# mattayes/tigerbeetle

Measured on AMD Instinct MI355X. Metric: transfers/sec committed (whole node, bit-exact results) + p99 batch latency, higher is better.
Workload: dtype u128

## Files before the change

### tigerbeetle_amd/csrc/engine.hip

```cpp
#include <hip/hip_runtime.h>

#include <algorithm>
#include <atomic>
#include <chrono>
#include <cmath>
#include <cstdarg>
#include <cstdio>
#include <cstdlib>
#include <cstring>
#include <numeric>
#include <string>
#include <vector>
#include <map>
#include <functional>
#include <mutex>

#include "../../include/tbgpu.h"
#include "../../include/tbgpu_bench.h"
#include "../../include/tbgpu_shard.h"
#include "k_apply.h"
#include "k_flow.h"
#include "k_aux.h"
#include "k_replay.h"
#include "k_route.h"
// ... 899 lines not shown
    if (E->wb.read_done) (void)hipEventDestroy(E->wb.read_done);
    if (E->wb.captured) (void)hipEventDestroy(E->wb.captured);
    for (hipEvent_t e : E->event_pool) (void)hipEventDestroy(e);
    if (E->pf_done) (void)hipEventDestroy(E->pf_done);
    for (int i = 0; i < 16; i++) if (E->markers[i]) (void)hipEventDestroy(E->markers[i]);
    if (E->stream) (void)hipStreamDestroy(E->stream);
    delete E;
}

extern "C" int tbgpu_reset(tbgpu_t* E) {
    API_ENTER(E, false);
    if (E->node) return node_api_reset(E->node);
    E->pf_input = E->pf_claim = nullptr;
    E->poisoned = false;
    HIPCK(hipSetDevice(E->device));
    if (E->wb.inflight) {
        HIPCK(hipStreamSynchronize(E->stream));
        HIPCK(hipStreamSynchronize(E->wb.stream));
        E->wb.inflight = E->wb.copying = E->wb.counts_known = E->wb.tail = false;
    }
    E->ckpt_valid = false;
    E->ckpt_scan = false;
    std::vector<u64>().swap(E->ckpt_ids);
    return engine_clear(E);
}

static int engine_sync(tbgpu* E) {
    HIPCK(hipMemcpyAsync(E->h_globals, E->g, sizeof(Globals), hipMemcpyDeviceToHost, E->stream));
    HIPCK(hipStreamSynchronize(E->stream));
    const Globals g = *E->h_globals;
    E->commit_ts = g.commit_timestamp;
    E->pending = false;
    int st = prof_collect(E);
    if (st) return st;
    if (g.panic) {
        E->poisoned = true;
        return fail(TBGPU_STATUS_PANIC, "device panic 0x%llx (the reference would have trapped)", (unsigned long long)g.panic);
    }
    return TBGPU_STATUS_OK;
}

static int enqueue_call(tbgpu* E, u8 op, u32 nb, const u64* h_off, const u8* events_dev, u32* results_dev,
                        u32* reply_bytes_dev, bool routed = false, u8* codes = nullptr, u32 cert_ext = 0,
                        const u8* events_src = nullptr, const u64* d_meta = nullptr,
                        const OwnerLegArgs* owner = nullptr, const u64* inline_meta = nullptr,
                        const NodeImport* imp = nullptr, const u64* ev_ts = nullptr) {
    const u64* d_off = d_meta ? d_meta : E->meta;
    const u64* d_ts = d_off + (nb + 1);
    u32 b0 = 0;
    while (b0 < nb) {
        u32 b1 = b0;
        while (b1 < nb && b1 - b0 < E->pb_max && h_off[b1 + 1] - h_off[b0] <= E->pe_max) b1++;
        if (b1 == b0) return fail(TBGPU_STATUS_INVALID, "batch larger than pass_events_max");
        const u64 n = h_off[b1] - h_off[b0];
        E->epoch++;
        if (E->epoch == 0) {
            HIPCK(hipMemsetAsync(E->T.account_mark, 0, E->account_cap * sizeof(u32), E->stream));
            E->epoch = 1;
            E->dedup_force = true;
        }
        PassArgs P{};
        P.op = op;
        P.epoch = E->epoch;
        P.b0 = b0;
        P.b1 = b1;
        P.e0 = h_off[b0];
        P.n = (u32)n;
        P.batch_off = d_off;
        P.batch_ts = d_ts;
        P.events = events_dev;
        P.events_src = events_src;
        P.results = results_dev;
        P.reply_bytes = reply_bytes_dev;
        P.info = E->info;
        P.eflags = E->eflags;
        P.dr = E->dr;
        P.cr = E->cr;
        P.ps = E->ps;
        P.rs = E->rs;
        P.amt = E->amt;
        P.amt_hi = E->amt + E->pe_max;
        P.kid = E->kid;
        P.kpid = E->kpid;
        P.dep_list = E->dep_list;
        P.dep_count = E->dep_count;
        P.dedup = E->dedup;
        P.dedup_mask = std::min<u64>(pow2_at_least(std::max<u64>(4 * n, 64)), E->dedup_cap) - 1;
        P.sum_shards = E->sum_shards;
        P.pass_words = E->sum_shards;
        P.log_base = E->log_next;
        P.T = E->T;
        P.ablate = E->ablate;
        P.routed = routed ? 1 : 0;
        P.codes = codes;
        P.cert_ext = cert_ext;
        P.seq_pv = E->balances_set ? 1u : 0u;
        P.ev_ts = ev_ts;
        P.inplace = E->inplace_call ? 1u : 0u;
        P.legs = (op == OP_CREATE_TRANSFERS && E->legs_ok && b1 - b0 <= LEG_PREPARES_MAX && n >= E->legs_min &&
                  !(E->ablate & ABL_LEGS) && !owner) ? 1 : 0;
        P.apply_late = (op == OP_CREATE_TRANSFERS && !P.legs) ? 1 : 0;
        P.leg_shift = E->leg_shift;
        P.leg_buckets = E->leg_buckets;
        P.resolve_slow = P.legs && E->lean_ok ? E->resolve_slow : nullptr;
        P.leg_w = E->leg_w;
        P.leg_off = E->leg_off;
        P.leg_tot = E->leg_tot;
        const bool flow = op == OP_CREATE_TRANSFERS && E->flow_ok && !E->balances_set && !(E->ablate & ABL_FLOW) &&
                          b1 - b0 <= FLOW_NB_MAX && !owner;
        P.flow_words = E->flow_ok ? E->F.words : nullptr;
        P.late_in_flow = (flow && (P.apply_late || P.legs)) ? 1u : 0u;

        P.kclock = nullptr;
        if (E->profile && !E->kclock_off && (E->prof_mask & ((1u << K_VALIDATE) | (1u << K_RESOLVE) | (1u << K_APPLY) | (1u << K_SPANS))) &&
            E->kclock_next < KCLOCK_SLOTS) {
            const u32 slot = E->kclock_next++;
            P.kclock = E->kclock + (u64)slot * KCLOCK_WORDS;
            E->kclock_used.push_back({slot, (n > 0 ? 1u : 0u) | 2u | (P.legs ? 4u : 0u)});
        }

        ProfilePair pass_pp;
        int st = prof_begin(E, &pass_pp, K_PASS);
        if (st) return st;
        ProfilePair pp;
        if ((st = prof_begin(E, &pp, K_CLEAR))) return st;
        const u64 clear_n = E->dedup_force ? E->dedup_cap : E->dedup_prev;
        const u32 clear_grid = (u32)std::min<u64>(1024, std::max<u64>(1, clear_n / 2048));
        u64* meta_dst = inline_meta && b0 == 0 ? (u64*)d_off : nullptr;
        ImportGate gate{};
        if (imp && n > 0) gate = ImportGate{imp->count, imp->room, 0, imp->flag};
        hipLaunchKernelGGL(tb_pass_clear, dim3(clear_grid), dim3(256), 0, E->stream, E->dedup, E->dedup_cap, E->sum_shards,
                           E->g, E->epoch, E->dedup_force ? 1u : 0u, E->leg_tot, E->leg_buckets, meta_dst,
                           inline_meta ? inline_meta[0] : 0, inline_meta ? inline_meta[1] : 0, inline_meta ? inline_meta[2] : 0,
                           P.kclock, gate, imp && b0 == 0 ? imp->leg_counts : nullptr,
                           imp && b0 == 0 ? imp->legs_n : 0u);
        HIPCK(hipGetLastError());
        E->dedup_force = false;
        E->dedup_prev = P.dedup_mask + 1;
        if ((st = prof_end(E, &pp))) return st;

        if (imp && n > 0) {
            const u32 ig = (u32)std::min<u64>(4096, (n + 255) / 256);
            hipLaunchKernelGGL(tb_node_import_flush, dim3((u32)std::min<u64>(1024, (E->account_cap + 255) / 256)), dim3(256), 0,
                               E->stream, E->T, E->account_cap, imp->N.world, imp->self, (const u32*)imp->flag);
            hipLaunchKernelGGL(tb_node_import, dim3(ig), dim3(256), 0, E->stream, E->T, imp->N, events_dev + P.e0 * 128, n,
                               imp->self, imp->count, imp->os_of);
            HIPCK(hipGetLastError());
        }
        if (n > 0) {
            if ((st = prof_begin(E, &pp, K_VALIDATE))) return st;
            const u32 grid = (u32)((n + VALIDATE_THREADS - 1) / VALIDATE_THREADS);
            if (op == OP_CREATE_TRANSFERS) {
                if (P.events_src) {
                    hipLaunchKernelGGL(tb_transfers_validate<true>, dim3(grid), dim3(VALIDATE_THREADS), 0, E->stream, P);
                } else {
                    hipLaunchKernelGGL(tb_transfers_validate<false>, dim3(grid), dim3(VALIDATE_THREADS), 0, E->stream, P);
                }
            } else {
                if (P.events_src) {
                    hipLaunchKernelGGL(tb_accounts_validate<true>, dim3(grid), dim3(VALIDATE_THREADS), 0, E->stream, P);
                } else {
                    hipLaunchKernelGGL(tb_accounts_validate<false>, dim3(grid), dim3(VALIDATE_THREADS), 0, E->stream, P);
                }
            }
            HIPCK(hipGetLastError());
            if (E->wb.copying) HIPCK(hipEventRecord(E->wb.read_done, E->stream));
            if ((st = prof_end(E, &pp))) return st;
        }
        if ((st = prof_begin(E, &pp, K_RESOLVE))) return st;
        if (op == OP_CREATE_TRANSFERS) {
            if (P.resolve_slow) {
                hipLaunchKernelGGL(tb_resolve_lean, dim3(b1 - b0), dim3(RESOLVE_THREADS), 0, E->stream, P);
            }
            hipLaunchKernelGGL(tb_resolve<OP_CREATE_TRANSFERS>, dim3(b1 - b0), dim3(RESOLVE_THREADS), 0, E->stream, P);
        } else {
            hipLaunchKernelGGL(tb_resolve<OP_CREATE_ACCOUNTS>, dim3(b1 - b0), dim3(RESOLVE_THREADS), 0, E->stream, P);
        }
        HIPCK(hipGetLastError());
        if ((st = prof_end(E, &pp))) return st;
        if (P.legs || P.apply_late) {
            if ((st = prof_begin(E, &pp, K_APPLY))) return st;
            if (P.legs) {
                hipLaunchKernelGGL(tb_apply_legs, dim3(E->leg_buckets + APPLY_EXTRA), dim3(APPLY_THREADS),
                                   tb_apply_lds_bytes(E->leg_shift, b1 - b0), E->stream, P);
            }
            if (n > 0 && !owner && !P.late_in_flow) {
                const u32 grid = (u32)std::min<u64>((n + 255) / 256, P.legs ? 2048 : 1u << 20);
                hipLaunchKernelGGL(tb_apply_events, dim3(grid), dim3(256), 0, E->stream, P);
            }
            HIPCK(hipGetLastError());
            if ((st = prof_end(E, &pp))) return st;
        }
        if ((st = prof_begin(E, &pp, K_REPLAY))) return st;
        if (flow) {
            UndoEntry* seq_undo = E->undo;
            u32 seq_cap = E->undo_cap;
            FlowArgs F = E->F;
            F.grid = flow_grid(E);

            if (n <= 65536) F.grid = std::min<u32>(F.grid, std::max<u32>(4, (u32)((n + 511) / 512)));
            if (E->flow_launch) F.grid = E->flow_launch;
            hipLaunchKernelGGL(tb_flow, dim3(F.grid), dim3(FLOW_THREADS), 0, E->stream, P, F, seq_undo, seq_cap);
        } else if (op == OP_CREATE_TRANSFERS) {
            hipLaunchKernelGGL(tb_replay<OP_CREATE_TRANSFERS>, dim3(1), dim3(REPLAY_THREADS), 0, E->stream, P,
                               E->undo, E->undo_cap);
        } else {
            hipLaunchKernelGGL(tb_replay<OP_CREATE_ACCOUNTS>, dim3(1), dim3(REPLAY_THREADS), 0, E->stream, P,
                               E->undo, E->undo_cap);
        }
        HIPCK(hipGetLastError());
        if ((st = prof_end(E, &pp))) return st;
        if (owner && n > 0) {
            hipLaunchKernelGGL(tb_owner_legs, dim3((u32)((n + 255) / 256)), dim3(256), 0, E->stream, P, *owner);
            HIPCK(hipGetLastError());
        }
        if (imp && imp->ev_legs) HIPCK(hipEventRecord((hipEvent_t)imp->ev_legs, E->stream));
        if ((st = prof_end(E, &pass_pp))) return st;
        E->passes++;
        E->events += n;
        if (op == OP_CREATE_TRANSFERS) E->log_next += n;
        b0 = b1;
    }
    return TBGPU_STATUS_OK;
}

static int prepare_call(tbgpu* E, u8 op, u32 nb, const u64* timestamps, const u32* lens, u64 floor_ts,
                        u64* total_events, bool upload = true) {
    if (op != OP_CREATE_ACCOUNTS && op != OP_CREATE_TRANSFERS) {
        return fail(TBGPU_STATUS_INVALID, "operation %u is not a create operation", op);
    }
    if (nb == 0) return fail(TBGPU_STATUS_INVALID, "no batches");
    if (nb > E->meta_cap) return fail(TBGPU_STATUS_INVALID, "too many batches in one call (%u > %llu)", nb,
                                      (unsigned long long)E->meta_cap);
    if (E->pending) {
        int st = engine_sync(E);
        if (st) return st;
    }
    u64* h_off = E->h_meta;
    u64* h_ts = E->h_meta + (nb + 1);
    u64 prev = floor_ts;
    h_off[0] = 0;
    for (u32 k = 0; k < nb; k++) {
        const u64 ts = timestamps[k];
        const u32 L = lens[k];
        if (L > BATCH_EVENTS_MAX) return fail(TBGPU_STATUS_INVALID, "batch %u has %u events (max %u)", k, L, BATCH_EVENTS_MAX);
        if (!(ts > prev)) return fail(TBGPU_STATUS_PANIC, "timestamp %llu <= commit timestamp %llu",
                                      (unsigned long long)ts, (unsigned long long)prev);
        if (L > 0) {
            if (ts < L) return fail(TBGPU_STATUS_PANIC, "timestamp %llu < batch length %u", (unsigned long long)ts, L);
            if (!(ts - L + 1 > prev)) return fail(TBGPU_STATUS_PANIC, "first event timestamp <= commit timestamp");
        }
        prev = ts;
        h_off[k + 1] = h_off[k] + L;
        h_ts[k] = ts;
    }
    if (op == OP_CREATE_TRANSFERS && E->log_next + h_off[nb] > E->xlog_cap) {
        return fail(TBGPU_STATUS_INVALID, "transfer log full (%llu + %llu events > capacity %llu)",
                    (unsigned long long)E->log_next, (unsigned long long)h_off[nb], (unsigned long long)E->xlog_cap);
    }
    if (upload) HIPCK(hipMemcpyAsync(E->meta, E->h_meta, (2 * (u64)nb + 1) * 8, hipMemcpyHostToDevice, E->stream));
    E->last_batch_ts = prev;
    *total_events = h_off[nb];
    return TBGPU_STATUS_OK;
}

static int commit_lookup(tbgpu* E, bool accounts, const void* input, uint32_t input_len, void* output,
                         uint32_t output_cap, uint32_t* out_len) {
    if (input_len % 16 != 0) return fail(TBGPU_STATUS_INVALID, "lookup body not a multiple of 16");
    const u32 n = input_len / 16;
    if (n > E->lookup_cap) return fail(TBGPU_STATUS_INVALID, "too many ids");
    if (n == 0) return TBGPU_STATUS_OK;
    HIPCK(hipMemcpyAsync(E->lookup_ids, input, input_len, hipMemcpyHostToDevice, E->stream));
    if (accounts) {
        hipLaunchKernelGGL(tb_lookup<true>, dim3((n + 255) / 256), dim3(256), 0, E->stream, E->T, E->lookup_ids, n,
                           E->lookup_out, E->lookup_found);
    } else {
        hipLaunchKernelGGL(tb_lookup<false>, dim3((n + 255) / 256), dim3(256), 0, E->stream, E->T, E->lookup_ids, n,
                           E->lookup_out, E->lookup_found);
    }
    HIPCK(hipGetLastError());
    std::vector<u8> found(n);
    std::vector<u8> recs((u64)n * 128);
    HIPCK(hipMemcpyAsync(found.data(), E->lookup_found, n, hipMemcpyDeviceToHost, E->stream));
    HIPCK(hipMemcpyAsync(recs.data(), E->lookup_out, (u64)n * 128, hipMemcpyDeviceToHost, E->stream));
    HIPCK(hipStreamSynchronize(E->stream));
    const u32 slots = output_cap / 128;
    u32 m = 0;
    for (u32 i = 0; i < n; i++) {
        if (found[i] && m < slots) {
            memcpy((u8*)output + (u64)m * 128, recs.data() + (u64)i * 128, 128);
            m++;
        }
    }
    *out_len = m * 128;
    return TBGPU_STATUS_OK;
}

static int wb_pump(tbgpu* E, u64 budget, hipEvent_t after);

static int commit_host(tbgpu* E, u8 op, u32 n, const uint64_t* timestamps, const void* const* inputs,
                       const uint32_t* input_lens, void* const* outputs, uint32_t* out_lens, const uint32_t* out_caps) {
    const void* claim = E->pf_claim;
    E->pf_claim = nullptr;
    std::vector<u32> lens(n);
    for (u32 k = 0; k < n; k++) {
        if (input_lens[k] % 128 != 0) return fail(TBGPU_STATUS_INVALID, "create body not a multiple of 128");
        lens[k] = input_lens[k] / 128;
        if (out_caps && (u64)out_caps[k] < (u64)lens[k] * 8) return fail(TBGPU_STATUS_INVALID, "output too small");
    }
// ... 2487 lines not shown
```

### tigerbeetle_amd/csrc/k_validate.h

```cpp
#pragma once

#include "pass.h"

#define TB_CODE_PANIC 63u

struct TransferScratch {
    u32 hz = 0;
    u32 dr = TB_NOT_FOUND, cr = TB_NOT_FOUND;
    u32 ps = TB_NOT_FOUND;
    u32 rs = TB_NOT_FOUND;
    u128 amount = 0;
    u128 contrib = 0;
    u64 kid = 0, kpid = 0;
    u64 rec_ts = 0;
};

__device__ static inline u32 tb_transfer_exists(const Transfer& t, const Transfer& e) {
    if (t.flags != e.flags) return CT_EXISTS_WITH_DIFFERENT_FLAGS;
    if (t.debit_account_id != e.debit_account_id) return CT_EXISTS_WITH_DIFFERENT_DEBIT_ACCOUNT_ID;
    if (t.credit_account_id != e.credit_account_id) return CT_EXISTS_WITH_DIFFERENT_CREDIT_ACCOUNT_ID;
    if (t.amount != e.amount) return CT_EXISTS_WITH_DIFFERENT_AMOUNT;
    if (t.user_data_128 != e.user_data_128) return CT_EXISTS_WITH_DIFFERENT_USER_DATA_128;
    if (t.user_data_64 != e.user_data_64) return CT_EXISTS_WITH_DIFFERENT_USER_DATA_64;
    if (t.user_data_32 != e.user_data_32) return CT_EXISTS_WITH_DIFFERENT_USER_DATA_32;
    if (t.timeout != e.timeout) return CT_EXISTS_WITH_DIFFERENT_TIMEOUT;
    if (t.code != e.code) return CT_EXISTS_WITH_DIFFERENT_CODE;
    return CT_EXISTS;
}

__device__ static inline u32 tb_post_void_exists(const Transfer& t, const Transfer& e, const Transfer& p) {
    if (t.flags != e.flags) return CT_EXISTS_WITH_DIFFERENT_FLAGS;
    if (t.amount == 0) {
        if (e.amount != p.amount) return CT_EXISTS_WITH_DIFFERENT_AMOUNT;
    } else {
        if (t.amount != e.amount) return CT_EXISTS_WITH_DIFFERENT_AMOUNT;
    }
    if (t.pending_id != e.pending_id) return CT_EXISTS_WITH_DIFFERENT_PENDING_ID;
    if (t.user_data_128 == 0) {
        if (e.user_data_128 != p.user_data_128) return CT_EXISTS_WITH_DIFFERENT_USER_DATA_128;
    } else {
        if (t.user_data_128 != e.user_data_128) return CT_EXISTS_WITH_DIFFERENT_USER_DATA_128;
    }
    if (t.user_data_64 == 0) {
        if (e.user_data_64 != p.user_data_64) return CT_EXISTS_WITH_DIFFERENT_USER_DATA_64;
    } else {
        if (t.user_data_64 != e.user_data_64) return CT_EXISTS_WITH_DIFFERENT_USER_DATA_64;
    }
    if (t.user_data_32 == 0) {
        if (e.user_data_32 != p.user_data_32) return CT_EXISTS_WITH_DIFFERENT_USER_DATA_32;
    } else {
        if (t.user_data_32 != e.user_data_32) return CT_EXISTS_WITH_DIFFERENT_USER_DATA_32;
    }
    return CT_EXISTS;
}

__device__ static inline Transfer tb_compose_post_void(const Transfer& t, const Transfer& p, u64 ts) {
    Transfer r;
    r.id = t.id;
    r.debit_account_id = p.debit_account_id;
    r.credit_account_id = p.credit_account_id;
    r.amount = t.amount > 0 ? t.amount : p.amount;
    r.pending_id = t.pending_id;
    r.user_data_128 = t.user_data_128 > 0 ? t.user_data_128 : p.user_data_128;
    r.user_data_64 = t.user_data_64 > 0 ? t.user_data_64 : p.user_data_64;
    r.user_data_32 = t.user_data_32 > 0 ? t.user_data_32 : p.user_data_32;
    r.timeout = 0;
    r.ledger = p.ledger;
    r.code = p.code;
    r.flags = t.flags;
    r.timestamp = ts;
    return r;
}

__device__ static inline u32 tb_claim_id(const PassArgs& P, const Transfer& t, u32 pe, TransferScratch& s,
                                         u32* exists_pos, u64 first = ~0ULL) {
    s.kid = tb_dedup_key(tb_lo(t.id), tb_hi(t.id));
    if (TB_ABL(P, ABL_SPEC)) return CLAIM_NEW;
    u32 entry = TB_NOT_FOUND;
    if (TB_ABL(P, ABL_CAS)) {
        s.rs = (u32)tb_xi_home(tb_lo(t.id), tb_hi(t.id), P.T.xidx_mask);
        s.hz |= HZ_SPEC;
        return CLAIM_NEW;
    }
    const u32 r = tb_transfer_claim(P.T, tb_lo(t.id), tb_hi(t.id), P.log_base + pe, P.log_base, exists_pos, &entry,
                                    first);
    if (r == CLAIM_NEW) {
        s.rs = entry;
        s.hz |= HZ_SPEC;
    } else if (r == CLAIM_COLLIDED) {
        s.hz |= HZ_SELFDEP;
        P.pass_words[PW_DUP] = 1;
    }
    return r;
}

__device__ static inline u32 tb_validate_post_void(const PassArgs& P, const Transfer& t, u64 ts, u32 pe,
                                                   TransferScratch& s) {
    const Tables& T = P.T;
    const u16 f = t.flags;
    if ((f & TF_POST) && (f & TF_VOID)) return CT_FLAGS_ARE_MUTUALLY_EXCLUSIVE;
    if (f & TF_PENDING) return CT_FLAGS_ARE_MUTUALLY_EXCLUSIVE;
    if (f & TF_BAL_DEBIT) return CT_FLAGS_ARE_MUTUALLY_EXCLUSIVE;
    if (f & TF_BAL_CREDIT) return CT_FLAGS_ARE_MUTUALLY_EXCLUSIVE;
    if (t.pending_id == 0) return CT_PENDING_ID_MUST_NOT_BE_ZERO;
    if (t.pending_id == TB_U128_MAX) return CT_PENDING_ID_MUST_NOT_BE_INT_MAX;
    if (t.pending_id == t.id) return CT_PENDING_ID_MUST_BE_DIFFERENT;
    if (t.timeout != 0) return CT_TIMEOUT_RESERVED_FOR_PENDING_TRANSFER;

    s.hz |= HZ_POSTVOID | HZ_PV_KEY;
    P.pass_words[PW_PV] = 1;
    s.kpid = tb_dedup_key(tb_lo(t.pending_id), tb_hi(t.pending_id));
    tb_dedup_mark(P);
    if (tb_dedup_insert(P.dedup, P.dedup_mask, s.kpid)) P.pass_words[PW_DUP] = 1;
    u32 es = TB_NOT_FOUND;
    const u32 claim = tb_claim_id(P, t, pe, s, &es);
    if (claim == CLAIM_COLLIDED) return R_OK;

    const u32 pslot = tb_transfer_find(T, tb_lo(t.pending_id), tb_hi(t.pending_id));
    if (pslot != TB_NOT_FOUND && (u64)pslot >= P.log_base) {
        s.hz |= HZ_SELFDEP;
        return R_OK;
    }
    if (pslot == TB_NOT_FOUND) return CT_PENDING_TRANSFER_NOT_FOUND;
    const Transfer p = T.xlog[pslot];
    if (!(p.flags & TF_PENDING)) return CT_PENDING_TRANSFER_NOT_PENDING;

    const u32 drs = tb_account_find(T, tb_lo(p.debit_account_id), tb_hi(p.debit_account_id));
    const u32 crs = tb_account_find(T, tb_lo(p.credit_account_id), tb_hi(p.credit_account_id));
    if (drs == TB_NOT_FOUND || crs == TB_NOT_FOUND) return TB_CODE_PANIC;

    if (t.debit_account_id > 0 && t.debit_account_id != p.debit_account_id) {
        return CT_PENDING_TRANSFER_HAS_DIFFERENT_DEBIT_ACCOUNT_ID;
    }
    if (t.credit_account_id > 0 && t.credit_account_id != p.credit_account_id) {
        return CT_PENDING_TRANSFER_HAS_DIFFERENT_CREDIT_ACCOUNT_ID;
    }
    if (t.ledger > 0 && t.ledger != p.ledger) return CT_PENDING_TRANSFER_HAS_DIFFERENT_LEDGER;
    if (t.code > 0 && t.code != p.code) return CT_PENDING_TRANSFER_HAS_DIFFERENT_CODE;

    const u128 amount = t.amount > 0 ? t.amount : p.amount;
    if (amount > p.amount) return CT_EXCEEDS_PENDING_TRANSFER_AMOUNT;
    if ((f & TF_VOID) && amount < p.amount) return CT_PENDING_TRANSFER_HAS_DIFFERENT_AMOUNT;

    if (claim == CLAIM_EXISTS) return tb_post_void_exists(t, T.xlog[es], p);

    const u8 posted = T.xposted[pslot];
    if (posted == POSTED_POSTED) return CT_PENDING_TRANSFER_ALREADY_POSTED;
    if (posted == POSTED_VOIDED) return CT_PENDING_TRANSFER_ALREADY_VOIDED;

    if (!(p.timestamp < ts)) return TB_CODE_PANIC;
    if (p.timeout > 0) {
        const u64 timeout_ns = (u64)p.timeout * 1000000000ULL;
        const u64 expiry = p.timestamp + timeout_ns;
        if (expiry < p.timestamp) return TB_CODE_PANIC;
        if (ts >= expiry) return CT_PENDING_TRANSFER_EXPIRED;
    }

    s.dr = drs;
    s.cr = crs;
    s.ps = pslot;
    s.hz |= HZ_ACCTS;
    if ((T.acct_hot[drs].flags | T.acct_hot[crs].flags) & AF_LIMITS) s.hz |= HZ_LIMIT;
    s.amount = (f & TF_POST) ? amount : 0;

    if ((s.hz & HZ_SPEC) && !P.inplace) T.xlog[P.log_base + pe] = tb_compose_post_void(t, p, ts);
    return R_OK;
}

__device__ static inline u32 tb_validate_transfer(const PassArgs& P, const Transfer& t, u64 ts, u32 pe,
                                                  TransferScratch& s) {
    const Tables& T = P.T;
    const u16 f = t.flags;
    if (f & TF_PADDING) return CT_RESERVED_FLAG;
    if (t.id == 0) return CT_ID_MUST_NOT_BE_ZERO;
    if (t.id == TB_U128_MAX) return CT_ID_MUST_NOT_BE_INT_MAX;

    if (f & (TF_POST | TF_VOID)) return tb_validate_post_void(P, t, ts, pe, s);

    if (t.debit_account_id == 0) return CT_DEBIT_ACCOUNT_ID_MUST_NOT_BE_ZERO;
    if (t.debit_account_id == TB_U128_MAX) return CT_DEBIT_ACCOUNT_ID_MUST_NOT_BE_INT_MAX;
    if (t.credit_account_id == 0) return CT_CREDIT_ACCOUNT_ID_MUST_NOT_BE_ZERO;
    if (t.credit_account_id == TB_U128_MAX) return CT_CREDIT_ACCOUNT_ID_MUST_NOT_BE_INT_MAX;
    if (t.credit_account_id == t.debit_account_id) return CT_ACCOUNTS_MUST_BE_DIFFERENT;
    if (t.pending_id != 0) return CT_PENDING_ID_MUST_BE_ZERO;
    if (!(f & TF_PENDING)) {
        if (t.timeout != 0) return CT_TIMEOUT_RESERVED_FOR_PENDING_TRANSFER;
    }
    if (!(f & (TF_BAL_DEBIT | TF_BAL_CREDIT))) {
        if (t.amount == 0) return CT_AMOUNT_MUST_NOT_BE_ZERO;
    }
    if (t.ledger == 0) return CT_LEDGER_MUST_NOT_BE_ZERO;
    if (t.code == 0) return CT_CODE_MUST_NOT_BE_ZERO;

    const u64 dlo = tb_lo(t.debit_account_id), dhi = tb_hi(t.debit_account_id);
    const u64 clo = tb_lo(t.credit_account_id), chi = tb_hi(t.credit_account_id);
    const u64 dpos = tb_hash_id(dlo, dhi) & T.account_mask;
    const u64 cpos = tb_hash_id(clo, chi) & T.account_mask;
    const u64 xpos = tb_xi_home(tb_lo(t.id), tb_hi(t.id), T.xidx_mask);
    const bool fake = TB_ABL(P, ABL_ACCTS);
    AccountHot d0 = {}, c0 = {};
    if (!fake) {
        d0 = T.acct_hot[dpos];
        c0 = T.acct_hot[cpos];
    }
    u64 x0 = ~0ULL;
    if (!TB_ABL(P, ABL_SPEC | ABL_CAS)) {
        x0 = tb_transfer_cas_home(T, tb_lo(t.id), tb_hi(t.id), (u32)(P.log_base + pe), xpos);
        if (x0 == 0) {
            s.rs = (u32)xpos;
            s.hz |= HZ_SPEC;
        }
    }
    AccountHot dr = {}, cr = {};
    u32 drs, crs;
    if (fake) {
        drs = (u32)(dlo & 1023);
        crs = (u32)(clo & 1023);
    } else {
        tb_account_find2(T, dlo, dhi, dpos, d0, clo, chi, cpos, c0, &drs, &crs, &dr, &cr);
    }
    u32 early = R_OK;
    if (drs == TB_NOT_FOUND) early = CT_DEBIT_ACCOUNT_NOT_FOUND;
    else if (crs == TB_NOT_FOUND) early = CT_CREDIT_ACCOUNT_NOT_FOUND;
    else if (!(ts > dr.timestamp) || !(ts > cr.timestamp)) early = TB_CODE_PANIC;
    else if (dr.ledger != cr.ledger) early = CT_ACCOUNTS_MUST_HAVE_THE_SAME_LEDGER;
    else if (t.ledger != dr.ledger) early = CT_TRANSFER_MUST_HAVE_THE_SAME_LEDGER_AS_ACCOUNTS;
    const bool balancing = (f & (TF_BAL_DEBIT | TF_BAL_CREDIT)) != 0;
    if (early == R_OK) {
        s.contrib = balancing && t.amount == 0 ? (u128)UINT64_MAX : t.amount;
        s.dr = drs;
        s.cr = crs;
        s.hz |= HZ_ACCTS;
        if ((dr.flags | cr.flags) & AF_LIMITS) s.hz |= HZ_LIMIT;
        if (balancing) {
            s.hz |= HZ_BAL;
            if (f & TF_BAL_DEBIT) P.T.account_mark[drs] = P.epoch;
            if (f & TF_BAL_CREDIT) P.T.account_mark[crs] = P.epoch;
            P.pass_words[PW_BAL] = 1;
        }
    }
    u32 es = TB_NOT_FOUND;
    const u32 claim = tb_claim_id(P, t, pe, s, &es, x0);
    if (early != R_OK) return early;
    if (claim == CLAIM_EXISTS) return tb_transfer_exists(t, T.xlog[es]);
    if (claim == CLAIM_COLLIDED || balancing) return R_OK;

    s.amount = t.amount;
    const u64 timeout_ns = (u64)t.timeout * 1000000000ULL;
    if (ts + timeout_ns < ts) return CT_OVERFLOWS_TIMEOUT;
    if ((s.hz & HZ_SPEC) && P.inplace) {
        s.hz |= HZ_INPLACE;
        P.T.xlog[P.log_base + pe].timestamp = ts;
    } else if ((s.hz & HZ_SPEC) && !TB_ABL(P, ABL_RECORD)) {
        s.rec_ts = ts;
        s.hz |= HZ_REC;
    }
    return R_OK;
}

template <bool SRC>
__global__ __launch_bounds__(VALIDATE_THREADS) void tb_transfers_validate(PassArgs P) {
    __shared__ __attribute__((aligned(16))) u8 stage[VALIDATE_THREADS * STAGE_STRIDE];

    const u32 tile0 = blockIdx.x * VALIDATE_THREADS;
    const u32 count = min((u32)VALIDATE_THREADS, P.n - tile0);
    const u32 pe = tile0 + threadIdx.x;
    const u64 e = P.e0 + pe;
    u32x4 tile[STAGE_CHUNKS];
    tb_stage_tile_issue<SRC>(P, tile0, count, tile, TB_ABL(P, EXP_NT));
    const LaneBatch B = tb_lane_batch(P, tile0, count, e, true);
    tb_stage_tile_commit<SRC>(P, tile0, count, tile, stage);

    TransferScratch s;
    if (threadIdx.x < count) {
        Transfer t = tb_read_staged<Transfer>(stage);
        const u32 L = (u32)(B.end - B.off);
        const u32 j = (u32)(e - B.off);
        u32 code;
        u64 routed_ts = 0;
        if (P.routed) {
            if (t.flags & (TF_LINKED | TF_POST | TF_VOID | TF_BAL_DEBIT | TF_BAL_CREDIT)) {
                tb_panic(P.T.g, PANIC_ASSERT);
            }
            routed_ts = t.timestamp;
            t.timestamp = 0;
        }
        if ((t.flags & TF_LINKED) && j == L - 1) {
            code = R_LINKED_EVENT_CHAIN_OPEN;
        } else if (t.timestamp != 0) {
            code = R_TIMESTAMP_MUST_BE_ZERO;
        } else {
            const u64 ts = P.routed ? routed_ts : P.ev_ts ? P.ev_ts[e] : B.ts - L + j + 1;
            code = tb_validate_transfer(P, t, ts, pe, s);
        }
        if (tb_hi(s.amount)) s.hz |= HZ_AMT_HI;
        P.info[pe] = code | s.hz;
        P.eflags[pe] = t.flags;
        P.dr[pe] = s.dr;
        P.cr[pe] = s.cr;
        if (s.hz & (HZ_POSTVOID | HZ_PV_KEY)) {
            P.ps[pe] = s.ps;
            P.kpid[pe] = s.kpid;
        }
        P.rs[pe] = s.rs;
        P.amt[pe] = tb_lo(s.amount);
        if (s.hz & HZ_AMT_HI) P.amt_hi[pe] = tb_hi(s.amount);
        if (code != R_OK) s.contrib = 0;
        if (s.rec_ts) *(u64*)(stage + tb_stage_off(threadIdx.x, 7) + 8) = s.rec_ts;
    }
    const u128 w = tb_wave_sum_u128(s.contrib);
    const u64 rec = __ballot(s.rec_ts != 0);
    const u32 lane = threadIdx.x & 63, w0 = threadIdx.x & ~63u;
    __builtin_amdgcn_fence(__ATOMIC_RELEASE, "wavefront");
    __builtin_amdgcn_wave_barrier();
    __builtin_amdgcn_fence(__ATOMIC_ACQUIRE, "wavefront");
#pragma unroll
    for (u32 r = 0; r < 8; r++) {
        const u32 c = lane + r * 64;
        const u32 row = c >> 3, part = c & 7;
        if ((rec >> row) & 1) {
            const u32x4 v = *(const u32x4*)(stage + tb_stage_off(w0 + row, part));
            u32x4* dst = (u32x4*)&P.T.xlog[P.log_base + tile0 + w0 + row] + part;
            if (TB_ABL(P, EXP_NT)) __builtin_nontemporal_store(v, dst);
            else *dst = v;
        }
    }
    __builtin_amdgcn_fence(__ATOMIC_RELEASE, "wavefront");
    __builtin_amdgcn_wave_barrier();
    if (lane == 0) {
        *(u64*)(stage + w0 * STAGE_STRIDE) = tb_lo(w);
        *(u64*)(stage + w0 * STAGE_STRIDE + 8) = tb_hi(w);
    }
    __syncthreads();
    if (threadIdx.x == 0) {
        u128 total = 0;
        for (u32 k = 0; k < VALIDATE_THREADS / 64; k++) {
            const u8* q = stage + k * 64 * STAGE_STRIDE;
            total = tb_sat_add(total, tb_u128(*(const u64*)q, *(const u64*)(q + 8)));
        }
        tb_sum_publish(P, total);
    }
}

__device__ static inline u32 tb_account_exists(const Account& a, const Account& e) {
    if (a.flags != e.flags) return CA_EXISTS_WITH_DIFFERENT_FLAGS;
    if (a.user_data_128 != e.user_data_128) return CA_EXISTS_WITH_DIFFERENT_USER_DATA_128;
    if (a.user_data_64 != e.user_data_64) return CA_EXISTS_WITH_DIFFERENT_USER_DATA_64;
    if (a.user_data_32 != e.user_data_32) return CA_EXISTS_WITH_DIFFERENT_USER_DATA_32;
    if (a.ledger != e.ledger) return CA_EXISTS_WITH_DIFFERENT_LEDGER;
    if (a.code != e.code) return CA_EXISTS_WITH_DIFFERENT_CODE;
    return CA_EXISTS;
}

__device__ static inline u32 tb_account_stateless(const Account& a) {
    if (a.reserved != 0) return CA_RESERVED_FIELD;
    if (a.flags & AF_PADDING) return CA_RESERVED_FLAG;
    if (a.id == 0) return CA_ID_MUST_NOT_BE_ZERO;
    if (a.id == TB_U128_MAX) return CA_ID_MUST_NOT_BE_INT_MAX;
    if ((a.flags & AF_DEBITS_MUST_NOT_EXCEED_CREDITS) && (a.flags & AF_CREDITS_MUST_NOT_EXCEED_DEBITS)) {
        return CA_FLAGS_ARE_MUTUALLY_EXCLUSIVE;
    }
    if (a.debits_pending != 0) return CA_DEBITS_PENDING_MUST_BE_ZERO;
    if (a.debits_posted != 0) return CA_DEBITS_POSTED_MUST_BE_ZERO;
    if (a.credits_pending != 0) return CA_CREDITS_PENDING_MUST_BE_ZERO;
    if (a.credits_posted != 0) return CA_CREDITS_POSTED_MUST_BE_ZERO;
    if (a.ledger == 0) return CA_LEDGER_MUST_NOT_BE_ZERO;
    if (a.code == 0) return CA_CODE_MUST_NOT_BE_ZERO;
    return R_OK;
}

template <bool SRC>
__global__ __launch_bounds__(VALIDATE_THREADS) void tb_accounts_validate(PassArgs P) {
    __shared__ __attribute__((aligned(16))) u8 stage[VALIDATE_THREADS * STAGE_STRIDE];
    const u32 tile0 = blockIdx.x * VALIDATE_THREADS;
    const u32 count = min((u32)VALIDATE_THREADS, P.n - tile0);
    const u32 pe = tile0 + threadIdx.x;
    const u64 e = P.e0 + pe;
    u32x4 tile[STAGE_CHUNKS];
    tb_stage_tile_issue<SRC>(P, tile0, count, tile);
    const LaneBatch B = tb_lane_batch(P, tile0, count, e, false);
    tb_stage_tile_commit<SRC>(P, tile0, count, tile, stage);
    if (threadIdx.x >= count) return;

    const Account a = tb_read_staged<Account>(stage);
    const u32 L = (u32)(B.end - B.off);
    const u32 j = (u32)(e - B.off);
    u32 code, hz = 0;
    u64 kid = 0;
    if ((a.flags & AF_LINKED) && j == L - 1) {
        code = R_LINKED_EVENT_CHAIN_OPEN;
    } else if (a.timestamp != 0) {
        code = R_TIMESTAMP_MUST_BE_ZERO;
    } else {
        code = tb_account_stateless(a);
        if (code == R_OK) {
            hz |= HZ_KEYS;
            kid = tb_dedup_key(tb_lo(a.id), tb_hi(a.id));
            tb_dedup_mark(P);
            if (tb_dedup_insert(P.dedup, P.dedup_mask, kid)) P.pass_words[PW_DUP] = 1;
            const u32 slot = tb_account_find(P.T, tb_lo(a.id), tb_hi(a.id));
            if (slot != TB_NOT_FOUND) code = tb_account_exists(a, tb_account_load(P.T, slot));
        }
    }
    P.info[pe] = code | hz;
    P.eflags[pe] = a.flags;
    P.kid[pe] = kid;
    P.kpid[pe] = 0;
}
```

### tigerbeetle_amd/csrc/pass.h

```cpp
#pragma once

#include "tb_device.h"

enum : u32 {
    HZ_KEYS = 1u << 8,
    HZ_LIMIT = 1u << 9,
    HZ_BAL = 1u << 10,
    HZ_ACCTS = 1u << 11,
    HZ_POSTVOID = 1u << 12,
    HZ_DEP = 1u << 13,
    HZ_EVAL_OK = 1u << 14,
    HZ_SPEC = 1u << 15,
    HZ_SELFDEP = 1u << 16,
    HZ_PV_KEY = 1u << 17,
    HZ_AMT_HI = 1u << 18,
    HZ_REC = 1u << 19,
    HZ_LATE = 1u << 20,
    HZ_INPLACE = 1u << 21,
};

#define SUM_SHARDS 64
#define FLOW_WORDS 16
#define VALIDATE_THREADS 256
#define RESOLVE_THREADS 1024
// ... 49 lines not shown

    u32* leg_off;
    u32* flow_words;
    u64* kclock;
};

#define KCLOCK_ENDS 16
#define KCLOCK_LINE 16
#define KCLOCK_STRIDE (KCLOCK_LINE * (1 + KCLOCK_ENDS))
#define KCLOCK_WORDS (3 * KCLOCK_STRIDE)
__device__ static inline void tb_kclock_stamp_end(u64* kernel_words) {
    atomicMax((unsigned long long*)(kernel_words + (1 + blockIdx.x % KCLOCK_ENDS) * KCLOCK_LINE),
              (unsigned long long)wall_clock64());
}
__device__ static inline void tb_kclock_start(const PassArgs& P, u32 k) {
    if (P.kclock && blockIdx.x < 8 && threadIdx.x == 0) {
        atomicMin((unsigned long long*)(P.kclock + k * KCLOCK_STRIDE), (unsigned long long)wall_clock64());
    }
}
__device__ static inline void tb_kclock_end(const PassArgs& P, u32 k) {
    if (!P.kclock) return;
    __syncthreads();
    if (threadIdx.x == 0) tb_kclock_stamp_end(P.kclock + k * KCLOCK_STRIDE);
}

enum : u32 { CERT_EXT_U128 = 1, CERT_EXT_U64 = 2 };

#ifndef LEG_SLOTS_MAX
#define LEG_SLOTS_MAX 1024
#endif
#ifndef LEG_BUCKETS_PREF
#define LEG_BUCKETS_PREF 2048
#endif
#define LEG_BUCKETS_MAX 4096
#define LEG_PREPARES_MAX 1024
#define LEG_SPLIT_MIN 65536
#define LEGS_MIN_EVENTS (1u << 18)
#ifndef APPLY_THREADS
#define APPLY_THREADS 256
#endif
#ifndef LEG_AMT_BITS
#define LEG_AMT_BITS 52
#endif
#define LEG_AMT_MASK ((1ULL << LEG_AMT_BITS) - 1)
static_assert((1u << (64 - LEG_AMT_BITS - 2)) >= LEG_SLOTS_MAX, "leg word: slot-in-bucket field too narrow");

__device__ static inline u64 tb_event_ts(const PassArgs& P, u32 b, u64 boff, u32 L, u32 i) {
    if (P.ev_ts) return P.ev_ts[boff + i];
    return P.routed ? *(const u64*)(P.events + (boff + i) * 128 + 120) : P.batch_ts[b] - L + 1 + i;
}
__device__ static inline bool tb_ts_carried(const PassArgs& P) { return P.routed || P.ev_ts; }

#ifdef TBGPU_TIMING_KNOBS
#define TB_ABL(P, bits) ((((P).ablate) & (bits)) != 0)
#else
#define TB_ABL(P, bits) false
#endif
enum : u32 { ABL_DEDUP = 1, ABL_SPEC = 2, ABL_ACCTS = 4, ABL_XFIND = 8, ABL_STAGE = 16, ABL_RECORD = 32, ABL_CAS = 64, EXP_NT = 128,
             ABL_LEGS = 256, ABL_LEG_STORES = 512, ABL_LEG_WORK = 1024,
             ABL_FLOW = 2048 };

__device__ static inline u32 tb_batch_search(const u64* off, u32 lo, u32 hi, u64 e) {
    while (hi - lo > 1) {
        const u32 mid = (lo + hi) >> 1;
        if (off[mid] <= e) lo = mid; else hi = mid;
    }
    return lo;
}

__device__ static inline u32 tb_tile_batch(const PassArgs& P, u64 e_first, u32 count, u64 e, u32* s_range) {
    if (threadIdx.x == 0) {
        s_range[0] = tb_batch_search(P.batch_off, P.b0, P.b1, e_first);
        s_range[1] = tb_batch_search(P.batch_off, s_range[0], P.b1, e_first + count - 1) + 1;
    }
    __syncthreads();
    return tb_batch_search(P.batch_off, s_range[0], s_range[1], e);
}

__device__ static inline u32 tb_wave_batch(const u64* off, u32 lo, u32 hi, u64 tile_e0, u32 count, u64 e) {
    const u32 w0 = (u32)__builtin_amdgcn_readfirstlane(threadIdx.x >> 6) * 64;
    if (w0 >= count) return lo;
    const u64 first = tile_e0 + w0, last = tile_e0 + min(count, w0 + 64) - 1;
    const u32 a = tb_batch_search(off, lo, hi, first);
    const u32 z = tb_batch_search(off, a, hi, last) + 1;
    return tb_batch_search(off, a, z, e);
}

#define STAGE_STRIDE 128
__device__ static inline u32 tb_stage_off(u32 row, u32 chunk) { return row * STAGE_STRIDE + ((chunk ^ (row & 7)) << 4); }
typedef unsigned int u32x4 __attribute__((ext_vector_type(4)));

#define STAGE_CHUNKS 8
__device__ static inline void tb_stage_issue(const u8* src, u32 count, u32x4 (&v)[STAGE_CHUNKS], bool nt = false) {
    const u32 last = count * 8 - 1;
#pragma unroll
    for (u32 r = 0; r < STAGE_CHUNKS; r++) {
        const u32 c = min(threadIdx.x + r * VALIDATE_THREADS, last);
        const u32x4* g = (const u32x4*)(src + (u64)c * 16);
        v[r] = nt ? __builtin_nontemporal_load(g) : *g;
    }
}
__device__ static inline void tb_stage_commit(const u32x4 (&v)[STAGE_CHUNKS], u32 count, u8* lds, u8* copy = nullptr) {
#pragma unroll
    for (u32 r = 0; r < STAGE_CHUNKS; r++) {
        const u32 c = threadIdx.x + r * VALIDATE_THREADS;
        const u32 ev = c >> 3, part = c & 7;
        if (ev < count) {
            *(u32x4*)(lds + tb_stage_off(ev, part)) = v[r];
            if (copy) *(u32x4*)(copy + (u64)c * 16) = v[r];
        }
    }
    __syncthreads();
}
__device__ static inline void tb_stage_events(const u8* src, u32 count, u8* lds) {
    u32x4 v[STAGE_CHUNKS];
    tb_stage_issue(src, count, v);
    tb_stage_commit(v, count, lds);
}

template <bool SRC>
__device__ static inline void tb_stage_tile_issue(const PassArgs& P, u32 tile0, u32 count, u32x4 (&v)[STAGE_CHUNKS],
                                                  bool nt = false) {
    const u64 off = (P.e0 + tile0) * 128;
    if (SRC) tb_stage_issue(P.events_src + off, count, v);
    else tb_stage_issue(P.events + off, count, v, nt);
}
template <bool SRC>
__device__ static inline void tb_stage_tile_commit(const PassArgs& P, u32 tile0, u32 count, const u32x4 (&v)[STAGE_CHUNKS],
                                                   u8* lds) {
    tb_stage_commit(v, count, lds, SRC ? const_cast<u8*>(P.events) + (P.e0 + tile0) * 128 : nullptr);
}

struct LaneBatch {
    u64 off, end;
    u64 ts;
};
__device__ static inline LaneBatch tb_lane_batch(const PassArgs& P, u32 tile0, u32 count, u64 e, bool want_ts) {
    const u32 b = tb_wave_batch(P.batch_off, P.b0, P.b1, P.e0 + tile0, count, e);
    LaneBatch B;
    B.off = P.batch_off[b];
    B.end = P.batch_off[b + 1];
    B.ts = want_ts && !tb_ts_carried(P) ? P.batch_ts[b] : 0;
    return B;
}

template <typename R>
__device__ static inline R tb_read_staged(const u8* lds) {
    R r;
#pragma unroll
    for (u32 k = 0; k < 8; k++) ((uint4*)&r)[k] = *(const uint4*)(lds + tb_stage_off(threadIdx.x, k));
    return r;
}

__device__ static inline u64 tb_wave_claim(bool take, u64* count, u64 k = 1) {
    const u64 m = __ballot(take);
    if (!m) return 0;
    const u32 lane = threadIdx.x & 63;
    const u32 leader = __ffsll((long long)m) - 1;
    u64 base = 0;
    if (lane == leader) base = atomicAdd((unsigned long long*)count, (unsigned long long)(k * __popcll(m)));
    base = __shfl(base, leader);
    return base + k * __popcll(m & ((1ULL << lane) - 1));
}

__device__ static inline u64 tb_wave_claim12(bool take, bool two, u64* count) {
    const u64 m = __ballot(take), m2 = __ballot(take && two);
    if (!m) return 0;
    const u32 lane = threadIdx.x & 63;
    const u32 leader = __ffsll((long long)m) - 1;
    u64 base = 0;
    if (lane == leader) base = atomicAdd((unsigned long long*)count, (unsigned long long)(__popcll(m) + __popcll(m2)));
    base = __shfl(base, leader);
    const u64 lt = (1ULL << lane) - 1;
    return base + __popcll(m & lt) + __popcll(m2 & lt);
}

__device__ static inline u128 tb_wave_sum_u128(u128 v) {
#pragma unroll
    for (int off = 32; off > 0; off >>= 1) {
        const u64 lo = __shfl_xor((unsigned long long)tb_lo(v), off);
        const u64 hi = __shfl_xor((unsigned long long)tb_hi(v), off);
        v = tb_sat_add(v, tb_u128(lo, hi));
    }
    return v;
}

#define PW_HUGE (2 * SUM_SHARDS)
#define PW_DUP (2 * SUM_SHARDS + 1)
#define PW_BAL (2 * SUM_SHARDS + 2)
#define PW_PV (2 * SUM_SHARDS + 3)
#define PW_LATE (2 * SUM_SHARDS + 4)
#define SUM_WORDS (2 * SUM_SHARDS + 5)
__device__ static inline void tb_sum_publish(const PassArgs& P, u128 block_sum) {
    if (block_sum == 0) return;
    if (tb_hi(block_sum) >> 36) {
        atomicOr((unsigned long long*)&P.sum_shards[PW_HUGE], 1ULL);
        return;
    }
    tb_atomic_add_u128(P.sum_shards + 2 * (blockIdx.x % SUM_SHARDS), block_sum);
}

__device__ static inline void tb_dedup_mark(const PassArgs& P) {
    P.T.g->dedup_dirty = ((u64)P.epoch << 8) | (u64)(64 - __clzll((long long)P.dedup_mask));
}

struct ImportGate {
    u64* count;
    u64 room, need;
    u32* flag;
};
__global__ __launch_bounds__(256) void tb_pass_clear(u64* dedup, u64 cap, u64* sum_shards, const Globals* g, u32 epoch,
                                                     u32 force, u32* leg_tot, u32 leg_buckets, u64* meta, u64 m0, u64 m1,
                                                     u64 m2, u64* kclock, ImportGate imp, u64* zero_b = nullptr,
                                                     u32 zero_b_n = 0) {
    const u64 w = g->dedup_dirty;
    if (blockIdx.x == 0 && threadIdx.x < SUM_WORDS) sum_shards[threadIdx.x] = 0;
    if (imp.count && blockIdx.x == 0 && threadIdx.x == 0) {
        const bool full = *imp.count + imp.need > imp.room;
        *imp.flag = full ? 1u : 0u;
        if (full) *imp.count = 0;
    }
    if (zero_b && blockIdx.x == 0 && threadIdx.x < zero_b_n) zero_b[threadIdx.x] = 0;
    if (kclock && blockIdx.x == 0) {
        for (u32 k = threadIdx.x; k < KCLOCK_WORDS; k += 256) kclock[k] = k % KCLOCK_STRIDE ? 0 : ~0ULL;
    }
    if (meta && blockIdx.x == 0 && threadIdx.x == 0) {
        meta[0] = m0;
        meta[1] = m1;
        meta[2] = m2;
    }
    if (blockIdx.x == 0 && leg_tot) {
        for (u32 k = threadIdx.x; k <= leg_buckets; k += 256) leg_tot[k] = 0;
    }
    u64 n = 0;
    if (force) n = cap;
    else if ((u32)(w >> 8) == epoch - 1 && w != 0) n = min(cap, 1ULL << (w & 255));
    typedef unsigned int v4 __attribute__((ext_vector_type(4)));
    const v4 z = {0, 0, 0, 0};
    for (u64 i = (u64)blockIdx.x * 256 + threadIdx.x; 2 * i < n; i += (u64)gridDim.x * 256) ((v4*)dedup)[i] = z;
    if (kclock && blockIdx.x == 0) {
        __syncthreads();
        if (threadIdx.x == 0) kclock[0] = wall_clock64();
    }
}

__device__ static inline u128 tb_sum_total(const u64* shards) {
    if (shards[PW_HUGE]) return TB_U128_MAX;
    u128 s = 0;
    for (int i = 0; i < SUM_SHARDS; i++) s = tb_sat_add(s, tb_u128(shards[2 * i], shards[2 * i + 1]));
    return s;
}

__device__ static inline u128 tb_sum_total_wave(const u64* shards) {
    static_assert(SUM_SHARDS == 64, "one shard per lane");
    if (shards[PW_HUGE]) return TB_U128_MAX;
    const u32 lane = threadIdx.x & 63;
    u64 lo = shards[2 * lane], hi = shards[2 * lane + 1];
    u32 sat = 0;
#pragma unroll
    for (u32 off = 1; off < 64; off <<= 1) {
        const u64 olo = __shfl_xor((unsigned long long)lo, off), ohi = __shfl_xor((unsigned long long)hi, off);
        sat |= __shfl_xor(sat, off);
        u128 r;
        sat |= tb_add_overflows(tb_u128(lo, hi), tb_u128(olo, ohi), &r) ? 1u : 0u;
        lo = tb_lo(r);
        hi = tb_hi(r);
    }
    const u32 l0 = __builtin_amdgcn_readfirstlane((u32)lo), l1 = __builtin_amdgcn_readfirstlane((u32)(lo >> 32));
    const u32 h0 = __builtin_amdgcn_readfirstlane((u32)hi), h1 = __builtin_amdgcn_readfirstlane((u32)(hi >> 32));
    if (__builtin_amdgcn_readfirstlane(sat)) return TB_U128_MAX;
    return tb_u128(((u64)l1 << 32) | l0, ((u64)h1 << 32) | h0);
}

__device__ static inline void tb_pass_cert(const PassArgs& P, u128& S, bool& cert_global, bool& cert64) {
    S = tb_sum_total_wave(P.sum_shards);
    u128 r;
    cert_global = S != TB_U128_MAX && !tb_add_overflows(tb_u128(P.T.g->bound_lo, P.T.g->bound_hi), S, &r);
    cert64 = cert_global && tb_hi(r) == 0;
    if (P.cert_ext) {
        cert_global = true;
        cert64 = P.cert_ext == CERT_EXT_U64;
    }
}

__device__ static inline u32 tb_block_excl_sum(u32 v, u32* s_wave, u32* total) {
    const u32 lane = threadIdx.x & 63, wave = threadIdx.x >> 6, nwaves = blockDim.x >> 6;
    u32 x = v;
#pragma unroll
    for (u32 off = 1; off < 64; off <<= 1) {
        const u32 o = __shfl_up(x, off);
        if (lane >= off) x += o;
    }
    if (lane == 63) s_wave[wave] = x;
    __syncthreads();
    u32 before = 0, tot = 0;
    for (u32 k = 0; k < nwaves; k++) {
        const u32 c = s_wave[k];
        before += k < wave ? c : 0;
        tot += c;
    }
    __syncthreads();
    *total = tot;
    return before + x - v;
}

template <typename T>
// ... 16 lines not shown
```

Baseline: 8.121 billion.

## Specialize transfer validation for in-place passes with half-size LDS staging

Adds an INPLACE template variant of the transfer validate kernel, selected when the pass is in-place and has no read-through source. That variant compiles out the record-timestamp writeback loop and the post/void xlog compose, and it transposes the 128-byte events through LDS in two 64-byte halves. This halves the shared-memory footprint per block, which should allow more resident blocks per CU. The cost is an extra __syncthreads, and a bug in the half-swizzle staging could corrupt events.

```diff
diff --git a/tigerbeetle_amd/csrc/engine.hip b/tigerbeetle_amd/csrc/engine.hip
--- a/tigerbeetle_amd/csrc/engine.hip
+++ b/tigerbeetle_amd/csrc/engine.hip
@@ -1075,9 +1075,11 @@
             const u32 grid = (u32)((n + VALIDATE_THREADS - 1) / VALIDATE_THREADS);
             if (op == OP_CREATE_TRANSFERS) {
                 if (P.events_src) {
-                    hipLaunchKernelGGL(tb_transfers_validate<true>, dim3(grid), dim3(VALIDATE_THREADS), 0, E->stream, P);
+                    hipLaunchKernelGGL((tb_transfers_validate<true, false>), dim3(grid), dim3(VALIDATE_THREADS), 0, E->stream, P);
+                } else if (P.inplace) {
+                    hipLaunchKernelGGL((tb_transfers_validate<false, true>), dim3(grid), dim3(VALIDATE_THREADS), 0, E->stream, P);
                 } else {
-                    hipLaunchKernelGGL(tb_transfers_validate<false>, dim3(grid), dim3(VALIDATE_THREADS), 0, E->stream, P);
+                    hipLaunchKernelGGL((tb_transfers_validate<false, false>), dim3(grid), dim3(VALIDATE_THREADS), 0, E->stream, P);
                 }
             } else {
                 if (P.events_src) {
diff --git a/tigerbeetle_amd/csrc/k_validate.h b/tigerbeetle_amd/csrc/k_validate.h
--- a/tigerbeetle_amd/csrc/k_validate.h
+++ b/tigerbeetle_amd/csrc/k_validate.h
@@ -94,6 +94,7 @@
     return r;
 }
 
+template <bool INPLACE>
 __device__ static inline u32 tb_validate_post_void(const PassArgs& P, const Transfer& t, u64 ts, u32 pe,
                                                    TransferScratch& s) {
     const Tables& T = P.T;
@@ -163,10 +164,13 @@
     if ((T.acct_hot[drs].flags | T.acct_hot[crs].flags) & AF_LIMITS) s.hz |= HZ_LIMIT;
     s.amount = (f & TF_POST) ? amount : 0;
 
-    if ((s.hz & HZ_SPEC) && !P.inplace) T.xlog[P.log_base + pe] = tb_compose_post_void(t, p, ts);
+    if constexpr (!INPLACE) {
+        if ((s.hz & HZ_SPEC) && !P.inplace) T.xlog[P.log_base + pe] = tb_compose_post_void(t, p, ts);
+    }
     return R_OK;
 }
 
+template <bool INPLACE>
 __device__ static inline u32 tb_validate_transfer(const PassArgs& P, const Transfer& t, u64 ts, u32 pe,
                                                   TransferScratch& s) {
     const Tables& T = P.T;
@@ -175,7 +179,7 @@
     if (t.id == 0) return CT_ID_MUST_NOT_BE_ZERO;
     if (t.id == TB_U128_MAX) return CT_ID_MUST_NOT_BE_INT_MAX;
 
-    if (f & (TF_POST | TF_VOID)) return tb_validate_post_void(P, t, ts, pe, s);
+    if (f & (TF_POST | TF_VOID)) return tb_validate_post_void<INPLACE>(P, t, ts, pe, s);
 
     if (t.debit_account_id == 0) return CT_DEBIT_ACCOUNT_ID_MUST_NOT_BE_ZERO;
     if (t.debit_account_id == TB_U128_MAX) return CT_DEBIT_ACCOUNT_ID_MUST_NOT_BE_INT_MAX;
@@ -248,19 +252,23 @@
     s.amount = t.amount;
     const u64 timeout_ns = (u64)t.timeout * 1000000000ULL;
     if (ts + timeout_ns < ts) return CT_OVERFLOWS_TIMEOUT;
-    if ((s.hz & HZ_SPEC) && P.inplace) {
+    if ((s.hz & HZ_SPEC) && (INPLACE || P.inplace)) {
         s.hz |= HZ_INPLACE;
         P.T.xlog[P.log_base + pe].timestamp = ts;
-    } else if ((s.hz & HZ_SPEC) && !TB_ABL(P, ABL_RECORD)) {
-        s.rec_ts = ts;
-        s.hz |= HZ_REC;
+    } else if constexpr (!INPLACE) {
+        if ((s.hz & HZ_SPEC) && !TB_ABL(P, ABL_RECORD)) {
+            s.rec_ts = ts;
+            s.hz |= HZ_REC;
+        }
     }
     return R_OK;
 }
 
-template <bool SRC>
+template <bool SRC, bool INPLACE>
 __global__ __launch_bounds__(VALIDATE_THREADS) void tb_transfers_validate(PassArgs P) {
-    __shared__ __attribute__((aligned(16))) u8 stage[VALIDATE_THREADS * STAGE_STRIDE];
+    static_assert(!(SRC && INPLACE), "an in-place pass has no read-through source");
+    constexpr u32 STRIDE = INPLACE ? STAGE_HALF_STRIDE : STAGE_STRIDE;
+    __shared__ __attribute__((aligned(16))) u8 stage[VALIDATE_THREADS * STRIDE];
 
     const u32 tile0 = blockIdx.x * VALIDATE_THREADS;
     const u32 count = min((u32)VALIDATE_THREADS, P.n - tile0);
@@ -269,11 +277,13 @@
     u32x4 tile[STAGE_CHUNKS];
     tb_stage_tile_issue<SRC>(P, tile0, count, tile, TB_ABL(P, EXP_NT));
     const LaneBatch B = tb_lane_batch(P, tile0, count, e, true);
-    tb_stage_tile_commit<SRC>(P, tile0, count, tile, stage);
+    Transfer t;
+    if constexpr (INPLACE) t = tb_stage_commit_halves<Transfer>(tile, count, stage);
+    else tb_stage_tile_commit<SRC>(P, tile0, count, tile, stage);
 
     TransferScratch s;
     if (threadIdx.x < count) {
-        Transfer t = tb_read_staged<Transfer>(stage);
+        if constexpr (!INPLACE) t = tb_read_staged<Transfer>(stage);
         const u32 L = (u32)(B.end - B.off);
         const u32 j = (u32)(e - B.off);
         u32 code;
@@ -291,7 +301,7 @@
             code = R_TIMESTAMP_MUST_BE_ZERO;
         } else {
             const u64 ts = P.routed ? routed_ts : P.ev_ts ? P.ev_ts[e] : B.ts - L + j + 1;
-            code = tb_validate_transfer(P, t, ts, pe, s);
+            code = tb_validate_transfer<INPLACE>(P, t, ts, pe, s);
         }
         if (tb_hi(s.amount)) s.hz |= HZ_AMT_HI;
         P.info[pe] = code | s.hz;
@@ -306,36 +316,40 @@
         P.amt[pe] = tb_lo(s.amount);
         if (s.hz & HZ_AMT_HI) P.amt_hi[pe] = tb_hi(s.amount);
         if (code != R_OK) s.contrib = 0;
-        if (s.rec_ts) *(u64*)(stage + tb_stage_off(threadIdx.x, 7) + 8) = s.rec_ts;
+        if constexpr (!INPLACE) {
+            if (s.rec_ts) *(u64*)(stage + tb_stage_off(threadIdx.x, 7) + 8) = s.rec_ts;
+        }
     }
     const u128 w = tb_wave_sum_u128(s.contrib);
-    const u64 rec = __ballot(s.rec_ts != 0);
     const u32 lane = threadIdx.x & 63, w0 = threadIdx.x & ~63u;
-    __builtin_amdgcn_fence(__ATOMIC_RELEASE, "wavefront");
-    __builtin_amdgcn_wave_barrier();
-    __builtin_amdgcn_fence(__ATOMIC_ACQUIRE, "wavefront");
+    if constexpr (!INPLACE) {
+        const u64 rec = __ballot(s.rec_ts != 0);
+        __builtin_amdgcn_fence(__ATOMIC_RELEASE, "wavefront");
+        __builtin_amdgcn_wave_barrier();
+        __builtin_amdgcn_fence(__ATOMIC_ACQUIRE, "wavefront");
 #pragma unroll
-    for (u32 r = 0; r < 8; r++) {
-        const u32 c = lane + r * 64;
-        const u32 row = c >> 3, part = c & 7;
-        if ((rec >> row) & 1) {
-            const u32x4 v = *(const u32x4*)(stage + tb_stage_off(w0 + row, part));
-            u32x4* dst = (u32x4*)&P.T.xlog[P.log_base + tile0 + w0 + row] + part;
-            if (TB_ABL(P, EXP_NT)) __builtin_nontemporal_store(v, dst);
-            else *dst = v;
+        for (u32 r = 0; r < 8; r++) {
+            const u32 c = lane + r * 64;
+            const u32 row = c >> 3, part = c & 7;
+            if ((rec >> row) & 1) {
+                const u32x4 v = *(const u32x4*)(stage + tb_stage_off(w0 + row, part));
+                u32x4* dst = (u32x4*)&P.T.xlog[P.log_base + tile0 + w0 + row] + part;
+                if (TB_ABL(P, EXP_NT)) __builtin_nontemporal_store(v, dst);
+                else *dst = v;
+            }
         }
     }
     __builtin_amdgcn_fence(__ATOMIC_RELEASE, "wavefront");
     __builtin_amdgcn_wave_barrier();
     if (lane == 0) {
-        *(u64*)(stage + w0 * STAGE_STRIDE) = tb_lo(w);
-        *(u64*)(stage + w0 * STAGE_STRIDE + 8) = tb_hi(w);
+        *(u64*)(stage + w0 * STRIDE) = tb_lo(w);
+        *(u64*)(stage + w0 * STRIDE + 8) = tb_hi(w);
     }
     __syncthreads();
     if (threadIdx.x == 0) {
         u128 total = 0;
         for (u32 k = 0; k < VALIDATE_THREADS / 64; k++) {
-            const u8* q = stage + k * 64 * STAGE_STRIDE;
+            const u8* q = stage + k * 64 * STRIDE;
             total = tb_sat_add(total, tb_u128(*(const u64*)q, *(const u64*)(q + 8)));
         }
         tb_sum_publish(P, total);
diff --git a/tigerbeetle_amd/csrc/pass.h b/tigerbeetle_amd/csrc/pass.h
--- a/tigerbeetle_amd/csrc/pass.h
+++ b/tigerbeetle_amd/csrc/pass.h
@@ -225,6 +225,32 @@
     return r;
 }
 
+#define STAGE_HALF_STRIDE 64
+__device__ static inline u32 tb_stage_half_off(u32 row, u32 chunk) {
+    return row * STAGE_HALF_STRIDE + ((chunk ^ ((row >> 2) & 3)) << 4);
+}
+template <typename R>
+__device__ static inline R tb_stage_commit_halves(const u32x4 (&v)[STAGE_CHUNKS], u32 count, u8* lds) {
+    static_assert(sizeof(R) == 128 && VALIDATE_THREADS == 256, "256 events of 128 B, eight chunks a thread");
+    const u32 part = threadIdx.x & 7, ev0 = threadIdx.x >> 3;
+    R rec;
+#pragma unroll
+    for (u32 h = 0; h < 2; h++) {
+        if (h) __syncthreads();
+        if ((part >> 2) == h) {
+#pragma unroll
+            for (u32 r = 0; r < STAGE_CHUNKS; r++) {
+                const u32 ev = ev0 + 32 * r;
+                if (ev < count) *(u32x4*)(lds + tb_stage_half_off(ev, part & 3)) = v[r];
+            }
+        }
+        __syncthreads();
+#pragma unroll
+        for (u32 k = 0; k < 4; k++) ((uint4*)&rec)[h * 4 + k] = *(const uint4*)(lds + tb_stage_half_off(threadIdx.x, k));
+    }
+    return rec;
+}
+
 __device__ static inline u64 tb_wave_claim(bool take, u64* count, u64 k = 1) {
     const u64 m = __ballot(take);
     if (!m) return 0;
```

Measured after the change: 8.449 billion, median of 6. 1.04x the previous value.
